# Sirui-Xu/InterDiff

Hardware: AMD Instinct MI355X
Metric: denoising frame-steps/sec (denoising-steps/sec x B x T frames) (higher is better)
Workload: dtype f32 (every contraction of the denoiser -- feed-forward block, QKV projection, self-attention, row-block contractions and the two token GEMMs: every fp32 operand as two f16 planes, 3 f16 MFMAs per product, fp32 accumulate; SMPL and everything else fp32 MFMA / VALU)

## Files before the change

### include/interdiff_hip.h

```cpp
#ifndef INTERDIFF_HIP_H
#define INTERDIFF_HIP_H

#include <stddef.h>
#include <stdint.h>

#ifdef __cplusplus
extern "C" {
#endif

#define IDF_OK            0
#define IDF_E_INVAL      -22
#define IDF_E_NOMEM      -12
#define IDF_E_LAUNCH     -5

int         interdiff_abi_version(void);
const char *interdiff_build_info(void);

int interdiff_rotation_6d_to_matrix   (const float *d6, float *m,  int64_t n, void *stream);
int interdiff_matrix_to_rotation_6d   (const float *m,  float *d6, int64_t n, void *stream);
int interdiff_matrix_to_axis_angle    (const float *m,  float *aa, int64_t n, void *stream);
int interdiff_axis_angle_to_matrix    (const float *aa, float *m,  int64_t n, void *stream);
int interdiff_axis_angle_to_quaternion(const float *aa, float *q,  int64_t n, void *stream);
int interdiff_rotation_6d_to_axis_angle(const float *d6, float *aa, int64_t n, void *stream);

// ... 160 lines not shown
size_t interdiff_correction_workspace_bytes(const idf_correction_ctx *c, int32_t B, int32_t T);
int interdiff_correction(const idf_correction_ctx *c, float *x0, const float *gt,
                         const float *hand_pose, const float *beta, const float *obj_points,
                         int32_t B, int32_t T, float blend_t ,
                         uint8_t *condition, int32_t *contact, float *distance, float *loss,
                         void *ws, size_t ws_bytes, void *stream);
int interdiff_correction_dev(const idf_correction_ctx *c, float *x0, const float *gt, const float *hand_pose,
                             const float *beta, const float *obj_points, int32_t B, int32_t T, const float *table,
                             const int64_t *state, void *ws, size_t ws_bytes, void *stream);

#define IDF_CONTACT_STATS 12
size_t interdiff_contact_nn_workspace_bytes(const idf_correction_ctx *c, int32_t B, int32_t T);
int interdiff_contact_nn(const idf_correction_ctx *c, const float *verts, const float *obj_points, const float *objR,
                         const float *objT, int32_t B, int32_t T, float *o2h, int32_t *idx, uint64_t *stats,
                         void *ws, size_t ws_bytes, void *stream);

size_t interdiff_metrics_workspace_bytes(const idf_correction_ctx *c, int32_t B, int32_t T);
int interdiff_metrics(const idf_correction_ctx *c, const float *obj_pred, const float *jtr,
                      const float *body_trans, const float *obj_gt, const float *jtr_gt,
                      const float *body_trans_gt, const float *verts, const float *obj_points,
                      int32_t B, int32_t T, int32_t J, float *out6 ,
                      void *ws, size_t ws_bytes, void *stream);

typedef struct {
    int32_t T, past_len, J, n_pre;
    const float *arena;
    int64_t dct_pad;
    int64_t dct;
    int64_t idct;
    int64_t layer[12];
// ... 113 lines not shown
```

### interdiff_amd/_lib.py

```python
import ctypes as C
import os
import torch

_HERE = os.path.dirname(os.path.abspath(__file__))
LIB_PATH = os.environ.get('INTERDIFF_HIP_LIB') or os.path.join(_HERE, 'csrc', 'libinterdiff_hip.so')
ABI_VERSION = 17

vp, i32, i64, f32, u64, sz = C.c_void_p, C.c_int32, C.c_int64, C.c_float, C.c_uint64, C.c_size_t

MDM_LAYERS = 8
FFN_SLICES = 5
STEP_EMBED_READY, STEP_EMBED_NEXT = 1, 2
LOSS_VAL, LOSS_TEST = 0, 1
TUNE = dict(ffn=3, ffn_math=4)


class SmplModel(C.Structure):
    _fields_ = [('V', i32), ('J', i32), ('n_betas', i32), ('KB', i32), ('S', i32),
                ('blend', vp), ('jt', vp), ('js', vp), ('parents', vp), ('skin_idx', vp), ('skin_w', vp)]


class MdmLayer(C.Structure):
    _fields_ = [('is_qan', i64),
                ('sa_in_w', i64), ('sa_in_b', i64), ('sa_out_w', i64), ('sa_out_b', i64),
# ... 91 lines not shown
    'interdiff_randn_at': (C.c_int, [vp, i64, u64, u64, u64, vp]),
    'interdiff_posterior_step_dev': (C.c_int, [vp, vp, vp, vp, i64, vp, vp, vp, i32, vp]),
    'interdiff_sampler_advance': (C.c_int, [vp, vp, i32, vp]),
    'interdiff_objprojector_sample': (C.c_int, [C.POINTER(ObjProj), vp, vp, vp, vp, i32, vp, vp]),
    'interdiff_objprojector_forward_workspace_bytes': (sz, [i32]),
    'interdiff_objprojector_forward': (C.c_int, [C.POINTER(ObjProj), vp, vp, vp, vp, i32, i32, vp, vp, sz, vp]),
    'interdiff_correction_workspace_bytes': (sz, [C.POINTER(CorrectionCtx), i32, i32]),
    'interdiff_correction': (C.c_int, [C.POINTER(CorrectionCtx), vp, vp, vp, vp, vp, i32, i32, f32,
                                       vp, vp, vp, vp, vp, sz, vp]),
    'interdiff_correction_dev': (C.c_int, [C.POINTER(CorrectionCtx), vp, vp, vp, vp, vp, i32, i32, vp, vp, vp, sz, vp]),
    'interdiff_metrics_workspace_bytes': (sz, [C.POINTER(CorrectionCtx), i32, i32]),
    'interdiff_metrics': (C.c_int, [C.POINTER(CorrectionCtx), vp, vp, vp, vp, vp, vp, vp, vp, i32, i32, i32,
                                    vp, vp, sz, vp]),
    'interdiff_contact_nn_workspace_bytes': (sz, [C.POINTER(CorrectionCtx), i32, i32]),
    'interdiff_contact_nn': (C.c_int, [C.POINTER(CorrectionCtx), vp, vp, vp, vp, i32, i32, vp, vp, vp, vp, sz, vp]),
    'interdiff_skeleton_objprojector_sample': (C.c_int, [C.POINTER(SkelObjProj), vp, vp, vp, i32, vp, vp, vp]),
    'interdiff_skeleton_correction': (C.c_int, [C.POINTER(SkelObjProj), vp, vp, vp, i32, i32, f32, vp, vp]),
    'interdiff_skeleton_metrics': (C.c_int, [vp, vp, vp, vp, vp, vp, i32, i32, i32, vp, vp]),
    'interdiff_skeleton_mdm_forward': (C.c_int, [C.POINTER(MdmWeights), C.POINTER(SkelHead), vp, vp, vp, vp, i32, i32, vp, vp, sz, vp]),
    'interdiff_skeleton_mdm_forward_step': (C.c_int, [C.POINTER(MdmWeights), C.POINTER(SkelHead), vp, vp, vp, vp, i32, i32, vp, vp, vp, vp, vp, sz, vp]),
    'interdiff_skeleton_mdm_encode_workspace_bytes': (sz, [i32, i32]),
    'interdiff_skeleton_mdm_encode': (C.c_int, [C.POINTER(MdmWeights), C.POINTER(SkelHead), vp, vp, i32, i32, vp, vp, sz, vp]),
    'interdiff_q_sample': (C.c_int, [vp, vp, vp, vp, vp, vp, i32, vp, vp, i32, i64, u64, u64, vp]),
    'interdiff_denoising_losses': (C.c_int, [vp, vp, i32, i32, i32, vp, vp]),
    'interdiff_sample_losses_workspace_bytes': (sz, [i32, i32]),
    'interdiff_sample_losses': (C.c_int, [vp, vp, vp, i32, i32, i32, i32, i32, vp, vp, vp, sz, vp]),
    'interdiff_correction_losses_workspace_bytes': (sz, [i32, i32, i32, i32]),
    'interdiff_correction_losses': (C.c_int, [vp, vp, vp, i32, vp, i32, i32, i32, i32, i32, i32, vp, vp, vp, sz, vp]),
    'interdiff_optimize_init': (C.c_int, [C.POINTER(OptCtx), C.POINTER(OptState), vp, vp, vp, vp, i32, vp]),
    'interdiff_optimize_loss_grad': (C.c_int, [C.POINTER(OptCtx), C.POINTER(OptState), vp]),
# ... 81 lines not shown
```

### interdiff_amd/correction.py

```python
import ctypes as C
import os
import itertools
import numpy as np
import torch
from . import _lib
from .geometry import MeshTopology

MARKERS67 = [3470, 3171, 3327, 857, 1812, 628, 182, 3116, 3040, 239,
             1666, 1725, 0, 2174, 1568, 1368, 3387, 2112, 1053, 1058,
             3336, 3346, 1323, 2108, 3122, 3314, 1252, 1082, 1861, 1454,
             850, 2224, 3233, 1769, 6728, 4343, 5273, 4116, 3694, 6399,
             6540, 6488, 3749, 5135, 5194, 3512, 5635, 5210, 4360, 4841,
             6786, 5573, 4538, 4544, 6736, 6747, 4804, 5568, 6544, 6682,
             5322, 4927, 5686, 4598, 6633, 3506, 3508]


_UID = itertools.count(1)


def correction_gate(t0):
    return not (t0 > 500 or t0 % 50 != 0)


class HipCorrection:
# ... 60 lines not shown
        hp, beta, pts = y['hand_pose'].contiguous().float(), y['beta'].contiguous().float(), y['obj_points'].contiguous().float()
        ws = self._workspace(B, T)
        dbg = [None] * 4
        if self.debug is not None:
            dbg = [torch.empty(B, dtype=torch.uint8, device=self.device), torch.empty(B, len(MARKERS67), dtype=torch.int32, device=self.device),
                   torch.empty(B, device=self.device), torch.empty(B, device=self.device)]
        blend_t = float(np.float32(t0) / np.float32(1000))
        _lib.check(self.lib.interdiff_correction(C.byref(self.ctx), _lib.dptr(x, torch.float32), _lib.dptr(gt, torch.float32),
                                                 _lib.dptr(hp), _lib.dptr(beta), _lib.dptr(pts), B, T, blend_t,
                                                 *[_lib.dptr(d, allow_none=True) for d in dbg], _lib.dptr(ws), ws.numel(),
                                                 _lib.stream()), 'correction')
        if self.debug is not None:
            self.debug.update(condition=dbg[0], contact=dbg[1], distance=dbg[2], loss=dbg[3])
        return x

    def contact_nn(self, verts, obj_points, objR, objT, want_stats=False):
        T, B = verts.shape[:2]
        P = self.ctx.n_points
        o2h = torch.empty(T, B, P, device=self.device)
        idx = torch.empty(T, B, P, dtype=torch.int32, device=self.device)
        stats = torch.zeros(12, dtype=torch.int64, device=self.device) if want_stats else None
        need = self.lib.interdiff_contact_nn_workspace_bytes(C.byref(self.ctx), B, T)
        ws = getattr(self, '_nn_ws', None)
        if ws is None or ws.numel() < need:
            ws = self._nn_ws = torch.empty(need, dtype=torch.uint8, device=self.device)
        v, pts, R_, t_ = (a.contiguous().float() for a in (verts, obj_points, objR, objT))
        _lib.check(self.lib.interdiff_contact_nn(C.byref(self.ctx), _lib.dptr(v), _lib.dptr(pts), _lib.dptr(R_), _lib.dptr(t_), B, T, _lib.dptr(o2h),
                                                 _lib.dptr(idx), _lib.dptr(stats, allow_none=True), _lib.dptr(ws), ws.numel(), _lib.stream()), 'contact_nn')
        return (o2h, idx, tuple(int(x) for x in stats.cpu())) if want_stats else (o2h, idx)

    def is_active(self, t0):
        return correction_gate(int(t0))

    def __call__(self, x, t, model_kwargs):
        t0 = getattr(t, 'host_value', None)
        if t0 is None:
            t0 = int(t[0])
        if not correction_gate(t0):
            return x
        return self.apply(x, t0, model_kwargs['y'])
```

### interdiff_amd/csrc/correction.hip

```cpp
#include "common.h"
#include "objproj.h"
#include "rot_math.h"
#include <float.h>

namespace {

constexpr int NBODY = 22;
constexpr int CTOK = 144;

__global__ __launch_bounds__(256) void corr_prepare_kernel(const float *__restrict__ x0, const float *__restrict__ gt,
                                                           const float *__restrict__ hand_pose, int B, int T,
                                                           float *__restrict__ pose, float *__restrict__ trans,
                                                           float *__restrict__ objR, float *__restrict__ objT,
                                                           float *__restrict__ gt_angles, float *__restrict__ gt_trans) {
    const int64_t i = (int64_t)blockIdx.x * 256 + threadIdx.x;
    const int64_t N = (int64_t)B * T;
    if (i >= N * 24) return;
    const int64_t n = i / 24;
    const int slot = (int)(i - n * 24), t = (int)(n / B), b = (int)(n - (int64_t)t * B);
    const float *xb = x0 + (size_t)b * CTOK * T + t;
    if (slot < NBODY) {
        float d[6], m[9], a[3];
#pragma unroll
        for (int k = 0; k < 6; ++k) d[k] = xb[(size_t)(slot * 6 + k) * T];
// ... 99 lines not shown
    }
#pragma unroll
    for (int k = 0; k < 2; ++k) {
        const int i = tid + 1024 * k;
        if (i < P) porder[(size_t)b * P + i] = (int32_t)(keys[i] & 2047u);
    }
}

constexpr int MAXM = 128;
constexpr float MARK_D2 = 0.00039999996079131961f;
constexpr int CB = 16;
constexpr int SB = 8;
constexpr int SEED_STRIDE = 4;
constexpr int CT = 1024;
constexpr int TASK = 64;
typedef float v2f __attribute__((ext_vector_type(2)));

struct ContactLds {
    int V4, nCB, nSB, nSeed;
    int rec, mark, box, sbox, seed, flags, red, pl, total;
    __host__ __device__ explicit ContactLds(int V) {
        V4 = (V + CB - 1) / CB * CB; nCB = V4 / CB; nSB = (nCB + SB - 1) / SB; nSeed = (nCB + SEED_STRIDE - 1) / SEED_STRIDE;
        rec = 0;
        mark = rec + V4;
        box = mark + MAXM;
        sbox = box + 3 * (nSB * SB / 2);
        seed = sbox + 3 * ((nSB + 2) / 2);
        flags = seed + 2 * ((nSeed + 1) / 2);
        red = flags + MAXM / 4;
        pl = red + CT / 4;
// ... 38 lines not shown
                                                          const int32_t *__restrict__ faces ,
                                                          const int32_t *__restrict__ adj_ptr,
                                                          const int32_t *__restrict__ adj_face,
                                                          const int32_t *__restrict__ adj_corner,
                                                          const int32_t *__restrict__ adj_pair ,
                                                          const int32_t *__restrict__ vorder ,
                                                          const int32_t *__restrict__ vrank ,
                                                          const int32_t *__restrict__ markers_pos , int M, int B,
                                                          float *__restrict__ markers_out, float *__restrict__ loss_sum,
                                                          float *__restrict__ min_dist, int32_t *__restrict__ label,
                                                          float *__restrict__ o2h_out ,
                                                          int32_t *__restrict__ idx_out ,
                                                          unsigned long long *__restrict__ stats ,
                                                          int64_t nn_from ,
                                                          const float *__restrict__ pts_frame , int frames_per_clip ,
                                                          const PredArgs pred) {
    extern __shared__ __attribute__((aligned(16))) float4 vs[];
    if constexpr (WITH_PRED) {
        if ((int)blockIdx.x < pred.nclips) {
            const int b = blockIdx.x, Tn = pred.op.T;
            for (int i = threadIdx.x; i < Tn * M; i += CT) {
                const int t = i / M, m = i - t * M;
                const size_t nfr = (size_t)t * B + b;
                const float *v = verts + (nfr * V + pred.markers_idx[m]) * 3;
                float *o = pred.markers + (nfr * M + m) * 3;
                o[0] = v[0]; o[1] = v[1]; o[2] = v[2];
            }
            __threadfence();
            __syncthreads();
            idf_objproj_dev::objproj_body<1>(reinterpret_cast<float *>(vs), pred.op, pred.obj_angles, pred.obj_trans, pred.markers, nullptr, B, b, pred.keep, nullptr);
            return;
        }
    }
    const ContactLds L(V);
    const int nCB = L.nCB, nSB = L.nSB;
    float4 *ms = vs + L.mark, *bb = vs + L.box, *sbb = vs + L.sbox, *sd = vs + L.seed;
    int *flags = reinterpret_cast<int *>(vs + L.flags);
    float *red = reinterpret_cast<float *>(vs + L.red);
    float *pl = reinterpret_cast<float *>(vs + L.pl);
    __shared__ int next_task;
    const int64_t n = WITH_PRED ? (int64_t)blockIdx.x - pred.nclips : (int64_t)blockIdx.x;
    const int b = OPT ? (int)(n / frames_per_clip) : (int)(n % B), tid = threadIdx.x;
    const float *vf = verts + (size_t)n * V * 3;
    const bool do_nn = n >= nn_from;
    long long t_prev = 0;
    int n_phase = 0;
    auto phase_done = [&]() {
        if (stats && tid == 0 && do_nn) {
            const long long now = (long long)__builtin_readcyclecounter();
            if (n_phase > 0) atomicAdd(stats + 3 + n_phase, (unsigned long long)(now - t_prev));
            t_prev = now;
        }
        ++n_phase;
    };
    phase_done();
    float R[9] = {1.f, 0.f, 0.f, 0.f, 1.f, 0.f, 0.f, 0.f, 1.f}, tr[3] = {0.f, 0.f, 0.f};
// ... 43 lines not shown
                typedef float f3v __attribute__((ext_vector_type(3), aligned(4)));
                const f3v pv = *reinterpret_cast<const f3v *>(vf + 3 * o[k]);
                x[k] = pv.x; y[k] = pv.y; z[k] = pv.z;
            }
        }
#pragma unroll
        for (int k = 0; k < 4; ++k) {
            const int v = v0 + k * CT;
            if (v < L.V4) {
                lds_rec_store(vs, v, x[k], y[k], z[k]);
                reinterpret_cast<int *>(vs + 2 * (v >> 1) + 1)[2 + (v & 1)] = o[k] >= 0 ? o[k] : 0x7fffffff;
            }
        }
    }
    if (tid < MAXM) flags[tid] = 0;
    const int ntask_all = (P + TASK - 1) / TASK;
    const int task0 = (int)((long long)blockIdx.y * ntask_all / gridDim.y), task1 = (int)((long long)(blockIdx.y + 1) * ntask_all / gridDim.y);
    if (tid == 0) next_task = task0;
    for (int i = tid; i < MAXP; i += CT) pl[i] = 0.f;
    __syncthreads();
    phase_done();
    if (!OPT && tid < ((M + 1) & ~1)) {
        float3 mk = make_float3(3e18f, 3e18f, 3e18f);
        if (tid < M) {
            mk = lds_rec(vs, my_marker_pos);
            if (markers_out) {
                float *mo = markers_out + ((size_t)n * M + tid) * 3;
                mo[0] = mk.x; mo[1] = mk.y; mo[2] = mk.z;
            }
        }
        lds_rec_store(ms, tid, mk.x, mk.y, mk.z);
// ... 21 lines not shown
            if ((lane_ & 7) == 0 && cb < nSB * SB) lds_box_store(bb, cb, make_float3(lx, ly, lz), make_float3(hx, hy, hz));
            const float slx = -wave_max(-lx), sly = -wave_max(-ly), slz = -wave_max(-lz), shx = wave_max(hx), shy = wave_max(hy), shz = wave_max(hz);
            if (lane_ == 0) lds_box_store(sbb, sb, make_float3(slx, sly, slz), make_float3(shx, shy, shz));
        }
#undef IDF_DPP8
        for (int k = tid; k < 2 * ((L.nSeed + 1) / 2); k += CT) {
            const float3 p = lds_rec(vs, min(k * SEED_STRIDE, nCB - 1) * CB);
            lds_rec_store(sd, k, p.x, p.y, p.z);
        }
    }
    const float *op = OPT ? pts_frame + (size_t)n * P * 3 : obj_points + (size_t)b * P * 3;
    const int ln = tid & 63, ntask = task1;
    __syncthreads();
    phase_done();
    float mind2 = FLT_MAX;
    unsigned n_exec = 0, n_test = 0, n_tasks = 0;
    for (;;) {
        int task = 0;
        if (ln == 0) task = atomicAdd(&next_task, 1);
        task = __builtin_amdgcn_readfirstlane(task);
        if (task >= ntask) break;
        ++n_tasks;
        const int sp = task * TASK + ln;
        const int i = sp < P ? (porder ? porder[(size_t)b * P + sp] : sp) : -1;
        const bool valid = i >= 0;
        float px = 0.f, py = 0.f, pz = 0.f;
        if (valid) { px = op[3 * i]; py = op[3 * i + 1]; pz = op[3 * i + 2]; }
        const float qx = OPT ? px : (px * R[0] + py * R[1] + pz * R[2]) + tr[0];
        const float qy = OPT ? py : (px * R[3] + py * R[4] + pz * R[5]) + tr[1];
        const float qz = OPT ? pz : (px * R[6] + py * R[7] + pz * R[8]) + tr[2];
        if (do_nn) {
#pragma clang fp contract(off)
            const v2f QX = v2f{qx, qx}, QY = v2f{qy, qy}, QZ = v2f{qz, qz};
            auto pair_d2 = [&](const float4 xy, const float4 zz) {
#pragma clang fp contract(off)
                const v2f dx = QX - v2f{xy.x, xy.y}, dy = QY - v2f{xy.z, xy.w}, dz = QZ - v2f{zz.x, zz.y};
                return (dx * dx + dy * dy) + dz * dz;
            };
            auto pair_a2 = [&](const float4 xy, const float2 zz) {
                const v2f dx = QX - v2f{xy.x, xy.y}, dy = QY - v2f{xy.z, xy.w}, dz = QZ - v2f{zz.x, zz.y};
                return __builtin_elementwise_fma(dz, dz, __builtin_elementwise_fma(dy, dy, dx * dx));
            };
            constexpr float SCAN_M = 1.000003814697265625f, SCAN_ABS = 1e-37f;
            float seed = FLT_MAX;
            for (int k = 0; k < (L.nSeed + 1) / 2; k += 4) {
                float4 xy[4]; float2 zz[4];
#pragma unroll
                for (int u = 0; u < 4; ++u) { xy[u] = sd[2 * min(k + u, (L.nSeed + 1) / 2 - 1)]; zz[u] = *reinterpret_cast<const float2 *>(&sd[2 * min(k + u, (L.nSeed + 1) / 2 - 1) + 1]); }
#pragma unroll
                for (int u = 0; u < 4; ++u) {
                    const v2f a2 = pair_a2(xy[u], zz[u]);
                    seed = fminf(fminf(seed, a2.x), a2.y);
                }
            }
            float thr = __builtin_fmaf(seed, SCAN_M, SCAN_ABS);
            float best = FLT_MAX, bthr = FLT_MAX;
            int tie = 0;
            int bblk = 0, bblk2 = 0;
            auto pair_lb = [&](const float4 a, const float4 bq, const float4 c) {
#pragma clang fp contract(off)
                const v2f ax = v2f{a.x, a.y} - QX, bx = QX - v2f{bq.z, bq.w};
                const v2f ay = v2f{a.z, a.w} - QY, by = QY - v2f{c.x, c.y};
                const v2f az = v2f{bq.x, bq.y} - QZ, bz = QZ - v2f{c.z, c.w};
                const v2f ex = v2f{fmaxf(fmaxf(ax.x, bx.x), 0.f), fmaxf(fmaxf(ax.y, bx.y), 0.f)};
                const v2f ey = v2f{fmaxf(fmaxf(ay.x, by.x), 0.f), fmaxf(fmaxf(ay.y, by.y), 0.f)};
                const v2f ez = v2f{fmaxf(fmaxf(az.x, bz.x), 0.f), fmaxf(fmaxf(az.y, bz.y), 0.f)};
                return __builtin_elementwise_fma(ez, ez, __builtin_elementwise_fma(ey, ey, ex * ex));
            };
            auto score_block = [&](int cb) {
                ++n_exec;
                const int v0 = cb * CB;
                float4 xy[CB / 2]; float2 zz[CB / 2];
#pragma unroll
                for (int u = 0; u < CB / 2; ++u) { xy[u] = vs[v0 + 2 * u]; zz[u] = *reinterpret_cast<const float2 *>(&vs[v0 + 2 * u + 1]); }
                float bm = FLT_MAX;
#pragma unroll
                for (int u = 0; u < CB / 2; ++u) {
                    const v2f a2 = pair_a2(xy[u], zz[u]);
                    bm = fminf(fminf(bm, a2.x), a2.y);
                }
                if (bm < best) {
                    const float w = __builtin_fmaf(bm, SCAN_M, SCAN_ABS);
                    if (best <= w) { tie = tie ? 2 : 1; bblk2 = bblk; } else tie = 0;
                    best = bm; bblk = v0; bthr = w; thr = fminf(thr, w);
                } else if (bm <= bthr) { tie = tie ? 2 : 1; bblk2 = v0; }
            };
            auto scan_super = [&](int sb) {
                const int cb0 = sb * SB;
#pragma unroll
                for (int j = 0; j < SB / 2; ++j) {
                    const int cb = cb0 + 2 * j;
                    const float4 *bx = bb + 3 * (cb >> 1);
                    const v2f lb = pair_lb(bx[0], bx[1], bx[2]);
                    n_test += 2;
                    if (__builtin_amdgcn_ballot_w64(valid && lb.x <= thr) != 0ull) score_block(cb);
                    if (__builtin_amdgcn_ballot_w64(valid && lb.y <= thr) != 0ull) score_block(cb + 1);
                }
            };
            if (!vorder) {
                for (int cb = 0; cb < nCB; ++cb) score_block(cb);
            } else
            for (int sb = 0; sb < nSB; sb += 2) {
                const float4 *bx = sbb + 3 * (sb >> 1);
                const v2f lb = pair_lb(bx[0], bx[1], bx[2]);
                n_test += 2;
                if (__builtin_amdgcn_ballot_w64(valid && lb.x <= thr) != 0ull) scan_super(sb);
                if (__builtin_amdgcn_ballot_w64(valid && lb.y <= thr) != 0ull) scan_super(sb + 1);
            }
            int pos = bblk, org = 0x7fffffff;
            float ebest = FLT_MAX;
            auto resolve_pair = [&](int pr) {
                const float4 xy = vs[2 * pr], zz = vs[2 * pr + 1];
                const v2f d2 = pair_d2(xy, zz);
                const int o0 = __builtin_bit_cast(int, zz.z), o1 = __builtin_bit_cast(int, zz.w);
                if (d2.x < ebest || (d2.x == ebest && o0 < org)) { ebest = d2.x; org = o0; pos = 2 * pr; }
                if (d2.y < ebest || (d2.y == ebest && o1 < org)) { ebest = d2.y; org = o1; pos = 2 * pr + 1; }
            };
            if (tie < 2) {
#pragma unroll
                for (int u = 0; u < CB / 2; ++u) resolve_pair((bblk >> 1) + u);
                if (tie) {
#pragma unroll
                    for (int u = 0; u < CB / 2; ++u) resolve_pair((bblk2 >> 1) + u);
                }
            } else {
                for (int pr = 0; pr < (V + 1) / 2; ++pr) resolve_pair(pr);
            }
            pos = min(pos, V - 1);
            if (org == 0x7fffffff) org = vorder ? vorder[pos] : pos;
            if constexpr (OPT) {
                if (valid) idx_out[(size_t)n * P + i] = org;
            } else if (valid) {
                const float3 v3 = lds_rec(vs, pos);
                float3 acc = make_float3(0.f, 0.f, 0.f);
                const int e0 = adj_ptr[org], e1 = adj_ptr[org + 1];
                if (adj_pair) {
                    for (int e = e0; e < e1; e += 4) {
                        int2 ab[4];
#pragma unroll
                        for (int u = 0; u < 4; ++u) ab[u] = *reinterpret_cast<const int2 *>(adj_pair + 2 * (size_t)min(e + u, e1 - 1));
#pragma unroll
                        for (int u = 0; u < 4; ++u) {
                            if (e + u < e1) {
                                const float3 nn = cross3(sub3(lds_rec(vs, ab[u].x), v3), sub3(lds_rec(vs, ab[u].y), v3));
                                acc.x += nn.x; acc.y += nn.y; acc.z += nn.z;
                            }
// ... 3 lines not shown
                    for (int e = e0; e < e1; ++e) {
                        const int f = adj_face[e], c = adj_corner[e];
                        const float3 p0 = lds_rec(vs, faces[3 * f]), p1 = lds_rec(vs, faces[3 * f + 1]), p2 = lds_rec(vs, faces[3 * f + 2]);
                        float3 nn;
                        if (c == 1) nn = cross3(sub3(p2, p1), sub3(p0, p1));
                        else if (c == 2) nn = cross3(sub3(p0, p2), sub3(p1, p2));
                        else nn = cross3(sub3(p1, p0), sub3(p2, p0));
                        acc.x += nn.x; acc.y += nn.y; acc.z += nn.z;
                    }
                }
                const float nl = fmaxf(sqrtf(acc.x * acc.x + acc.y * acc.y + acc.z * acc.z), 1e-6f);
                const float vx = qx - v3.x, vy = qy - v3.y, vz = qz - v3.z;
                const float dt = (acc.x / nl) * vx + (acc.y / nl) * vy + (acc.z / nl) * vz;
                const float d = sqrtf(vx * vx + vy * vy + vz * vz);
                const float o2h = d * (dt > 0.f ? 1.f : (dt < 0.f ? -1.f : 0.f));
                if (o2h_out) o2h_out[(size_t)n * P + i] = o2h;
                if (idx_out) idx_out[(size_t)n * P + i] = org;
                pl[sp] = o2h < 0.f ? fabsf(o2h) * 20.0f : 0.f;
            }
        }
        if (!OPT && valid) {
#pragma clang fp contract(off)
            const v2f QX = v2f{qx, qx}, QY = v2f{qy, qy}, QZ = v2f{qz, qz};
            for (int p2 = 0; p2 < (M + 1) / 2; ++p2) {
                const float4 xy = ms[2 * p2], zz = ms[2 * p2 + 1];
                const v2f dx = v2f{xy.x, xy.y} - QX, dy = v2f{xy.z, xy.w} - QY, dz = v2f{zz.x, zz.y} - QZ;
                const v2f d2 = __builtin_elementwise_fma(dy, dy, dx * dx) + dz * dz;
                mind2 = fminf(fminf(mind2, d2.x), d2.y);
                if (__builtin_amdgcn_ballot_w64(fminf(d2.x, d2.y) < MARK_D2) != 0ull) {
                    if (d2.x < MARK_D2) flags[2 * p2] = 1;
                    if (d2.y < MARK_D2) flags[2 * p2 + 1] = 1;
                }
            }
        }
    }
    if (stats && ln == 0 && do_nn) {
        atomicAdd(stats, (unsigned long long)n_exec);
        atomicAdd(stats + 1, (unsigned long long)nCB * n_tasks);
        atomicAdd(stats + 2, (unsigned long long)n_test);
    }
    phase_done();
    if constexpr (OPT) return;
    __syncthreads();
    phase_done();
    float loss = 0.f;
#pragma unroll
    for (int k = 0; k < MAXP / CT; ++k) loss += pl[tid + CT * k];
    red[tid] = loss;
    __syncthreads();
    for (int s = CT / 2; s > 0; s >>= 1) {
        if (tid < s) red[tid] += red[tid + s];
        __syncthreads();
    }
    const float loss_total = red[0];
// ... 5 lines not shown
        __syncthreads();
    }
    if (tid == 0) { loss_sum[n] = loss_total; min_dist[n] = red[0] == FLT_MAX ? FLT_MAX : sqrtf(red[0]); }
    if (tid < M) label[(size_t)n * M + tid] = flags[tid];
    phase_done();
    if (stats && tid == 0 && do_nn) atomicAdd(stats + 3, 1ull);
}

size_t contact_lds_bytes(int V) { return (size_t)ContactLds(V).total * sizeof(float4); }

int launch_contact(hipStream_t s, int64_t N, const float *verts, int V, const float *obj_points, int P, int32_t *porder,
                   const float *objR, const float *objT, const idf_correction_ctx *c, int B, float *markers, float *loss_sum,
                   float *min_dist, int32_t *label, float *o2h, int32_t *idx, unsigned long long *stats, int64_t nn_from, const PredArgs *pred = nullptr) {
    const int M = c->n_markers;
    const size_t lds = contact_lds_bytes(V);
    if (lds > 160 * 1024 - 16384 || P > MAXP) return IDF_E_INVAL;
    const bool ordered = c->vorder != nullptr;
    if (ordered != (c->faces_scan != nullptr) || ordered != (c->markers_scan != nullptr) || ordered != (c->adj_pair_scan != nullptr)) return IDF_E_INVAL;
    const int32_t *faces = ordered ? c->faces_scan : c->faces, *mpos = ordered ? c->markers_scan : c->markers_idx;
    if (porder) hipLaunchKernelGGL(corr_point_order_kernel, dim3((unsigned)B), dim3(1024), 0, s, obj_points, P, porder);
    if (pred) {
        const size_t lds2 = (pred->nclips > 0 && lds < idf_objproj_dev::OBJPROJ_LDS) ? idf_objproj_dev::OBJPROJ_LDS : lds;
        static std::atomic<uint64_t> lds_ok2{0};
        if (lds2 > 160 * 1024 - 2048) return IDF_E_INVAL;
        if (idf_opt_in_lds(reinterpret_cast<const void *>(corr_contact_kernel<false, true>), 160 * 1024 - 2048, lds_ok2) != IDF_OK) return IDF_E_LAUNCH;
        hipLaunchKernelGGL((corr_contact_kernel<false, true>), dim3((unsigned)(N + pred->nclips)), dim3(CT), lds2, s, verts, V, obj_points, P, porder, objR, objT, faces,
                           c->adj_ptr, c->adj_face, c->adj_corner, c->adj_pair_scan, c->vorder, c->vrank, mpos, M, B, markers, loss_sum, min_dist, label, o2h, idx,
                           stats, nn_from, nullptr, 0, *pred);
        return IDF_OK;
    }
    static std::atomic<uint64_t> lds_ok{0};
    if (idf_opt_in_lds(reinterpret_cast<const void *>(corr_contact_kernel<false>), 160 * 1024 - 16384, lds_ok) != IDF_OK) return IDF_E_LAUNCH;
    hipLaunchKernelGGL(corr_contact_kernel<false>, dim3((unsigned)N), dim3(CT), lds, s, verts, V, obj_points, P, porder, objR, objT, faces,
                       c->adj_ptr, c->adj_face, c->adj_corner, c->adj_pair_scan, c->vorder, c->vrank, mpos, M, B, markers, loss_sum, min_dist, label, o2h, idx,
                       stats, nn_from, nullptr, 0, PredArgs{});
    return IDF_OK;
}

__global__ __launch_bounds__(128) void corr_reduce_kernel(const float *__restrict__ loss_sum, const float *__restrict__ min_dist,
                                                          const int32_t *__restrict__ label, int B, int T, int past, int P, int M,
                                                          uint8_t *__restrict__ condition, int32_t *__restrict__ contact,
                                                          float *__restrict__ distance_out, float *__restrict__ loss_out) {
    extern __shared__ float fr[];
    const int b = blockIdx.x, tid = threadIdx.x;
    for (int t = tid; t < T; t += 128) {
        fr[t] = loss_sum[(size_t)t * B + b];
        fr[T + t] = min_dist[(size_t)t * B + b];
    }
    if (tid < M) {
        int c = 0;
// ... 129 lines not shown
    }
    if (valid) near[(size_t)n * V + vid] = hit ? 1 : 0;
}

}

int idf_point_order(hipStream_t s, const float *obj_points, int B, int P, int32_t *porder) {
    if (P > MAXP) return IDF_E_INVAL;
    hipLaunchKernelGGL(corr_point_order_kernel, dim3((unsigned)B), dim3(1024), 0, s, obj_points, P, porder);
    return IDF_OK;
}

int idf_nn_scan_opt(hipStream_t s, int64_t N, int frames_per_clip, const float *verts, int V, const float *pts_frame, const float *obj_points, int P,
                    const int32_t *porder, const idf_correction_ctx *c, int32_t *yidx) {
    const size_t lds = contact_lds_bytes(V);
    if (lds > 160 * 1024 - 16384 || P > MAXP || !c->vorder) return IDF_E_INVAL;
    const int B = (int)(N / frames_per_clip);
    static std::atomic<uint64_t> lds_ok{0};
    if (idf_opt_in_lds(reinterpret_cast<const void *>(corr_contact_kernel<true>), 160 * 1024 - 16384, lds_ok) != IDF_OK) return IDF_E_LAUNCH;
    hipLaunchKernelGGL(corr_contact_kernel<true>, dim3((unsigned)N, 2), dim3(CT), lds, s, verts, V, obj_points, P, porder, nullptr, nullptr, nullptr,
                       nullptr, nullptr, nullptr, nullptr, c->vorder, c->vrank, nullptr, 0, B, nullptr, nullptr, nullptr, nullptr, nullptr, yidx, nullptr, (int64_t)0,
                       pts_frame, frames_per_clip, PredArgs{});
    return IDF_OK;
}

int idf_near_mask_opt(hipStream_t s, int64_t N, int frames_per_clip, const float *verts, int V, const float *pts_frame, int P, const int32_t *porder,
                      const int32_t *vorder, float *psort, float *pbox, int32_t *near) {
    if (P > MAXP || !vorder) return IDF_E_INVAL;
    hipLaunchKernelGGL(opt_patch_kernel, dim3((unsigned)N), dim3(256), 0, s, pts_frame, P, porder, frames_per_clip, reinterpret_cast<float4 *>(psort),
                       reinterpret_cast<float4 *>(pbox));
    hipLaunchKernelGGL(opt_near_kernel, dim3((unsigned)idf_cdiv(V, 256), (unsigned)N), dim3(256), 0, s, verts, V, P, reinterpret_cast<const float4 *>(psort),
                       reinterpret_cast<const float4 *>(pbox), vorder, near);
    return IDF_OK;
}

namespace {

}

extern "C" size_t interdiff_correction_workspace_bytes(const idf_correction_ctx *c, int32_t B, int32_t T) {
    if (!c || !c->smpl || B <= 0 || T <= 0) return 0;
    return carve(c, B, T, nullptr).total;
}

static int correction_impl(const idf_correction_ctx *c, float *x0, const float *gt, const float *hand_pose,
                           const float *beta, const float *obj_points, int32_t B, int32_t T, float blend_t, const float *blend_table,
                           const int64_t *blend_state, uint8_t *condition, int32_t *contact, float *distance, float *loss, void *ws,
                           size_t ws_bytes, void *stream) {
    if (!c || !c->smpl || !c->objproj || !x0 || !gt || !hand_pose || !beta || !obj_points || !ws || B <= 0 || T <= 0) return IDF_E_INVAL;
    const int V = c->smpl->V, M = c->n_markers, P = c->n_points;
    if (c->smpl->J != 52 || c->smpl->n_betas != 10 || M > MAXM || M != c->objproj->P || P > MAXP || T != c->objproj->T ||
        c->past_len != c->objproj->past_len || c->past_len >= T)
        return IDF_E_INVAL;
    CorrWs w = carve(c, B, T, ws);
    if (ws_bytes < w.total) return IDF_E_NOMEM;
    hipStream_t s = idf_stream(stream);
    const int64_t N = (int64_t)B * T;
    const bool fused = (c->tune & 2) == 0 && idf_objproj_check(c->objproj) == IDF_OK;
    idf_prof_mark(IDF_K_CORR_PREPARE, s);
    hipLaunchKernelGGL(corr_prepare_kernel, dim3((unsigned)idf_cdiv(N * 24, 256)), dim3(256), 0, s, x0, gt, hand_pose, B, T, w.pose,
                       w.trans, w.objR, w.objT, w.gt_angles, w.gt_trans);
    int rc = interdiff_smpl_forward(c->smpl, w.pose, beta, w.trans, N, w.verts, w.jtr, nullptr, w.smpl_ws, w.smpl_ws_bytes, stream);
    if (rc) return rc;
    idf_prof_mark(IDF_K_CORR_CONTACT, s);
    PredArgs pred{};
    if (fused) {
        pred.op = *c->objproj;
// ... 145 lines not shown
    if (!c || B <= 0 || T <= 0) return 0;
    return carve_metrics(c, B, T, nullptr).total;
}

extern "C" int interdiff_contact_nn(const idf_correction_ctx *c, const float *verts, const float *obj_points, const float *objR,
                                    const float *objT, int32_t B, int32_t T, float *o2h, int32_t *idx, uint64_t *stats, void *ws,
                                    size_t ws_bytes, void *stream) {
    if (!c || !c->smpl || !verts || !obj_points || !objR || !objT || !ws || B <= 0 || T <= 0 || (!o2h && !idx)) return IDF_E_INVAL;
    if (c->n_markers > MAXM || c->n_points > MAXP) return IDF_E_INVAL;
    MetWs w = carve_metrics(c, B, T, ws);
    if (ws_bytes < w.total) return IDF_E_NOMEM;
    hipStream_t s = idf_stream(stream);
    if (stats && hipMemsetAsync(stats, 0, IDF_CONTACT_STATS * sizeof(uint64_t), s) != hipSuccess) return IDF_E_LAUNCH;
    const int rc = launch_contact(s, (int64_t)B * T, verts, c->smpl->V, obj_points, c->n_points, w.porder, objR, objT, c, B, w.markers, w.loss_sum,
                                  w.min_dist, w.label, o2h ? o2h : w.o2h, idx, reinterpret_cast<unsigned long long *>(stats), 0);
    if (rc) return rc;
    IDF_CHECK_LAUNCH();
    return IDF_OK;
}

extern "C" size_t interdiff_metrics_workspace_bytes(const idf_correction_ctx *c, int32_t B, int32_t T) {
    if (!c || B <= 0 || T <= 0) return 0;
    return carve_metrics(c, B, T, nullptr).total;
}

extern "C" int interdiff_metrics(const idf_correction_ctx *c, const float *obj_pred, const float *jtr, const float *body_trans,
                                 const float *obj_gt, const float *jtr_gt, const float *body_trans_gt, const float *verts,
                                 const float *obj_points, int32_t B, int32_t T, int32_t J, float *out6, void *ws, size_t ws_bytes,
                                 void *stream) {
    if (!c || !c->smpl || !obj_pred || !jtr || !body_trans || !obj_gt || !jtr_gt || !body_trans_gt || !verts || !obj_points || !out6 ||
// ... 20 lines not shown
```

Measured before the change: 7.317 million.

## Split each contact nearest-neighbour query across two lanes with DPP reductions

Adds a two-lane mode, on by default, to the contact kernel. Each object point is handled by a lane pair: the seed scan, block scoring and exhaustive rescans are split between the two lanes, and the partial minima and argmins are combined through DPP swaps. This halves the points per task and aims to shorten the serial per-point scan and cut divergence, at the cost of more ballots and cross-lane shuffles. The change also reorders workgroups so that nearest-neighbour frames launch first, raises the opt-in LDS limit, adds runner and rescan statistics, and exposes a standalone contact_nn_opt entry point.

```diff
diff --git a/include/interdiff_hip.h b/include/interdiff_hip.h
--- a/include/interdiff_hip.h
+++ b/include/interdiff_hip.h
@@ -198,6 +198,9 @@
 int interdiff_contact_nn(const idf_correction_ctx *c, const float *verts, const float *obj_points, const float *objR,
                          const float *objT, int32_t B, int32_t T, float *o2h, int32_t *idx, uint64_t *stats,
                          void *ws, size_t ws_bytes, void *stream);
+
+int interdiff_contact_nn_opt(const idf_correction_ctx *c, const float *verts, const float *pts_frame, const float *obj_points, int32_t B,
+                             int32_t T, int32_t *porder, int32_t *idx, void *stream);
 
 size_t interdiff_metrics_workspace_bytes(const idf_correction_ctx *c, int32_t B, int32_t T);
 int interdiff_metrics(const idf_correction_ctx *c, const float *obj_pred, const float *jtr,
diff --git a/interdiff_amd/_lib.py b/interdiff_amd/_lib.py
--- a/interdiff_amd/_lib.py
+++ b/interdiff_amd/_lib.py
@@ -129,6 +129,7 @@
                                     vp, vp, sz, vp]),
     'interdiff_contact_nn_workspace_bytes': (sz, [C.POINTER(CorrectionCtx), i32, i32]),
     'interdiff_contact_nn': (C.c_int, [C.POINTER(CorrectionCtx), vp, vp, vp, vp, i32, i32, vp, vp, vp, vp, sz, vp]),
+    'interdiff_contact_nn_opt': (C.c_int, [C.POINTER(CorrectionCtx), vp, vp, vp, i32, i32, vp, vp, vp]),
     'interdiff_skeleton_objprojector_sample': (C.c_int, [C.POINTER(SkelObjProj), vp, vp, vp, i32, vp, vp, vp]),
     'interdiff_skeleton_correction': (C.c_int, [C.POINTER(SkelObjProj), vp, vp, vp, i32, i32, f32, vp, vp]),
     'interdiff_skeleton_metrics': (C.c_int, [vp, vp, vp, vp, vp, vp, i32, i32, i32, vp, vp]),
diff --git a/interdiff_amd/correction.py b/interdiff_amd/correction.py
--- a/interdiff_amd/correction.py
+++ b/interdiff_amd/correction.py
@@ -98,7 +98,7 @@
             self.debug.update(condition=dbg[0], contact=dbg[1], distance=dbg[2], loss=dbg[3])
         return x
 
-    def contact_nn(self, verts, obj_points, objR, objT, want_stats=False):
+    def contact_nn(self, verts, obj_points, objR, objT, want_stats=False, want_frames=False):
         T, B = verts.shape[:2]
         P = self.ctx.n_points
         o2h = torch.empty(T, B, P, device=self.device)
@@ -111,7 +111,29 @@
         v, pts, R_, t_ = (a.contiguous().float() for a in (verts, obj_points, objR, objT))
         _lib.check(self.lib.interdiff_contact_nn(C.byref(self.ctx), _lib.dptr(v), _lib.dptr(pts), _lib.dptr(R_), _lib.dptr(t_), B, T, _lib.dptr(o2h),
                                                  _lib.dptr(idx), _lib.dptr(stats, allow_none=True), _lib.dptr(ws), ws.numel(), _lib.stream()), 'contact_nn')
-        return (o2h, idx, tuple(int(x) for x in stats.cpu())) if want_stats else (o2h, idx)
+        out = (o2h, idx)
+        if want_stats:
+            out += (tuple(int(x) for x in stats.cpu()),)
+        if want_frames:
+            N, M, al = T * B, self.ctx.n_markers, lambda x: (x + 255) // 256 * 256
+            off = al(N * 36) + al(N * 12) + al(N * P * 4) + al(N * M * 12)
+            loss_sum = ws[off:off + N * 4].view(torch.float32).reshape(T, B).clone()
+            off += al(N * 4)
+            min_dist = ws[off:off + N * 4].view(torch.float32).reshape(T, B).clone()
+            off += al(N * 4)
+            label = ws[off:off + N * M * 4].view(torch.int32).reshape(T, B, M).clone()
+            out += (dict(loss_sum=loss_sum, min_dist=min_dist, label=label),)
+        return out
+
+    def contact_nn_opt(self, verts, pts_frame, obj_points):
+        B, T = verts.shape[:2]
+        P = self.ctx.n_points
+        idx = torch.empty(B, T, P, dtype=torch.int32, device=self.device)
+        porder = torch.empty(B, P, dtype=torch.int32, device=self.device)
+        v, pf, pts = (a.contiguous().float() for a in (verts, pts_frame, obj_points))
+        _lib.check(self.lib.interdiff_contact_nn_opt(C.byref(self.ctx), _lib.dptr(v), _lib.dptr(pf), _lib.dptr(pts), B, T, _lib.dptr(porder), _lib.dptr(idx),
+                                                     _lib.stream()), 'contact_nn_opt')
+        return idx
 
     def is_active(self, t0):
         return correction_gate(int(t0))
diff --git a/interdiff_amd/csrc/correction.hip b/interdiff_amd/csrc/correction.hip
--- a/interdiff_amd/csrc/correction.hip
+++ b/interdiff_amd/csrc/correction.hip
@@ -137,6 +137,7 @@
 constexpr int SEED_STRIDE = 4;
 constexpr int CT = 1024;
 constexpr int TASK = 64;
+constexpr size_t CONTACT_LDS_MAX = 160 * 1024 - 2048;
 typedef float v2f __attribute__((ext_vector_type(2)));
 
 struct ContactLds {
@@ -205,6 +206,7 @@
                                                           unsigned long long *__restrict__ stats ,
                                                           int64_t nn_from ,
                                                           const float *__restrict__ pts_frame , int frames_per_clip ,
+                                                          int two_lane ,
                                                           const PredArgs pred) {
     extern __shared__ __attribute__((aligned(16))) float4 vs[];
     if constexpr (WITH_PRED) {
@@ -230,7 +232,9 @@
     float *red = reinterpret_cast<float *>(vs + L.red);
     float *pl = reinterpret_cast<float *>(vs + L.pl);
     __shared__ int next_task;
-    const int64_t n = WITH_PRED ? (int64_t)blockIdx.x - pred.nclips : (int64_t)blockIdx.x;
+    const int64_t wg = WITH_PRED ? (int64_t)blockIdx.x - pred.nclips : (int64_t)blockIdx.x;
+    const int64_t n_frames = (int64_t)gridDim.x - (WITH_PRED ? pred.nclips : 0), n_scan = n_frames - nn_from;
+    const int64_t n = (nn_from > 0 && n_scan > 0) ? (wg < n_scan ? wg + nn_from : wg - n_scan) : wg;
     const int b = OPT ? (int)(n / frames_per_clip) : (int)(n % B), tid = threadIdx.x;
     const float *vf = verts + (size_t)n * V * 3;
     const bool do_nn = n >= nn_from;
@@ -304,7 +308,8 @@
         }
     }
     if (tid < MAXM) flags[tid] = 0;
-    const int ntask_all = (P + TASK - 1) / TASK;
+    const int task_pts = two_lane ? TASK / 2 : TASK;
+    const int ntask_all = (P + task_pts - 1) / task_pts;
     const int task0 = (int)((long long)blockIdx.y * ntask_all / gridDim.y), task1 = (int)((long long)(blockIdx.y + 1) * ntask_all / gridDim.y);
     if (tid == 0) next_task = task0;
     for (int i = tid; i < MAXP; i += CT) pl[i] = 0.f;
@@ -356,14 +361,18 @@
     __syncthreads();
     phase_done();
     float mind2 = FLT_MAX;
-    unsigned n_exec = 0, n_test = 0, n_tasks = 0;
+    unsigned n_exec = 0, n_test = 0, n_tasks = 0, n_runner = 0, n_rescan = 0;
+    const int hl = two_lane ? (ln & 1) : 0;
+    const unsigned long long lanes_first = two_lane ? 0x5555555555555555ull : ~0ull;
+    auto other_f = [](float v) { return __builtin_bit_cast(float, __builtin_amdgcn_update_dpp(0, __builtin_bit_cast(int, v), 0xB1, 0xf, 0xf, false)); };
+    auto other_i = [](int v) { return __builtin_amdgcn_update_dpp(0, v, 0xB1, 0xf, 0xf, false); };
     for (;;) {
         int task = 0;
         if (ln == 0) task = atomicAdd(&next_task, 1);
         task = __builtin_amdgcn_readfirstlane(task);
         if (task >= ntask) break;
         ++n_tasks;
-        const int sp = task * TASK + ln;
+        const int sp = two_lane ? task * (TASK / 2) + (ln >> 1) : task * TASK + ln;
         const int i = sp < P ? (porder ? porder[(size_t)b * P + sp] : sp) : -1;
         const bool valid = i >= 0;
         float px = 0.f, py = 0.f, pz = 0.f;
@@ -385,7 +394,7 @@
             };
             constexpr float SCAN_M = 1.000003814697265625f, SCAN_ABS = 1e-37f;
             float seed = FLT_MAX;
-            for (int k = 0; k < (L.nSeed + 1) / 2; k += 4) {
+            auto seed_group = [&](int k) {
                 float4 xy[4]; float2 zz[4];
 #pragma unroll
                 for (int u = 0; u < 4; ++u) { xy[u] = sd[2 * min(k + u, (L.nSeed + 1) / 2 - 1)]; zz[u] = *reinterpret_cast<const float2 *>(&sd[2 * min(k + u, (L.nSeed + 1) / 2 - 1) + 1]); }
@@ -394,6 +403,12 @@
                     const v2f a2 = pair_a2(xy[u], zz[u]);
                     seed = fminf(fminf(seed, a2.x), a2.y);
                 }
+            };
+            if (two_lane) {
+                for (int k = 4 * hl; k < (L.nSeed + 1) / 2; k += 8) seed_group(k);
+                seed = fminf(seed, other_f(seed));
+            } else {
+                for (int k = 0; k < (L.nSeed + 1) / 2; k += 4) seed_group(k);
             }
             float thr = __builtin_fmaf(seed, SCAN_M, SCAN_ABS);
             float best = FLT_MAX, bthr = FLT_MAX;
@@ -409,23 +424,40 @@
                 const v2f ez = v2f{fmaxf(fmaxf(az.x, bz.x), 0.f), fmaxf(fmaxf(az.y, bz.y), 0.f)};
                 return __builtin_elementwise_fma(ez, ez, __builtin_elementwise_fma(ey, ey, ex * ex));
             };
-            auto score_block = [&](int cb) {
-                ++n_exec;
-                const int v0 = cb * CB;
-                float4 xy[CB / 2]; float2 zz[CB / 2];
-#pragma unroll
-                for (int u = 0; u < CB / 2; ++u) { xy[u] = vs[v0 + 2 * u]; zz[u] = *reinterpret_cast<const float2 *>(&vs[v0 + 2 * u + 1]); }
-                float bm = FLT_MAX;
-#pragma unroll
-                for (int u = 0; u < CB / 2; ++u) {
-                    const v2f a2 = pair_a2(xy[u], zz[u]);
-                    bm = fminf(fminf(bm, a2.x), a2.y);
-                }
+            auto block_scored = [&](float bm, int v0) {
                 if (bm < best) {
                     const float w = __builtin_fmaf(bm, SCAN_M, SCAN_ABS);
                     if (best <= w) { tie = tie ? 2 : 1; bblk2 = bblk; } else tie = 0;
                     best = bm; bblk = v0; bthr = w; thr = fminf(thr, w);
                 } else if (bm <= bthr) { tie = tie ? 2 : 1; bblk2 = v0; }
+            };
+            auto score_block = [&](int cb) {
+                ++n_exec;
+                const int v0 = cb * CB;
+                float4 xy[CB / 2]; float2 zz[CB / 2];
+#pragma unroll
+                for (int u = 0; u < CB / 2; ++u) { xy[u] = vs[v0 + 2 * u]; zz[u] = *reinterpret_cast<const float2 *>(&vs[v0 + 2 * u + 1]); }
+                float bm = FLT_MAX;
+#pragma unroll
+                for (int u = 0; u < CB / 2; ++u) {
+                    const v2f a2 = pair_a2(xy[u], zz[u]);
+                    bm = fminf(fminf(bm, a2.x), a2.y);
+                }
+                block_scored(bm, v0);
+            };
+            auto score_block2 = [&](int cb) {
+                ++n_exec;
+                const int v0 = cb * CB, h0 = v0 + (CB / 2) * hl;
+                float4 xy[CB / 4]; float2 zz[CB / 4];
+#pragma unroll
+                for (int u = 0; u < CB / 4; ++u) { xy[u] = vs[h0 + 2 * u]; zz[u] = *reinterpret_cast<const float2 *>(&vs[h0 + 2 * u + 1]); }
+                float bm = FLT_MAX;
+#pragma unroll
+                for (int u = 0; u < CB / 4; ++u) {
+                    const v2f a2 = pair_a2(xy[u], zz[u]);
+                    bm = fminf(fminf(bm, a2.x), a2.y);
+                }
+                block_scored(fminf(bm, other_f(bm)), v0);
             };
             auto scan_super = [&](int sb) {
                 const int cb0 = sb * SB;
@@ -439,8 +471,35 @@
                     if (__builtin_amdgcn_ballot_w64(valid && lb.y <= thr) != 0ull) score_block(cb + 1);
                 }
             };
+            constexpr unsigned long long EVEN = 0x5555555555555555ull, ODD = 0xaaaaaaaaaaaaaaaaull;
+            auto scan_super2 = [&](int sb) {
+                const int cb0 = sb * SB;
+#pragma unroll
+                for (int j = 0; j < SB / 4; ++j) {
+                    const int cb = cb0 + 4 * j;
+                    const float4 *bx = bb + 3 * ((cb >> 1) + hl);
+                    const v2f lb = pair_lb(bx[0], bx[1], bx[2]);
+                    n_test += 4;
+                    if ((__builtin_amdgcn_ballot_w64(valid && lb.x <= thr) & EVEN) != 0ull) score_block2(cb);
+                    if ((__builtin_amdgcn_ballot_w64(valid && lb.y <= thr) & EVEN) != 0ull) score_block2(cb + 1);
+                    if ((__builtin_amdgcn_ballot_w64(valid && lb.x <= thr) & ODD) != 0ull) score_block2(cb + 2);
+                    if ((__builtin_amdgcn_ballot_w64(valid && lb.y <= thr) & ODD) != 0ull) score_block2(cb + 3);
+                }
+            };
             if (!vorder) {
-                for (int cb = 0; cb < nCB; ++cb) score_block(cb);
+                if (two_lane) for (int cb = 0; cb < nCB; ++cb) score_block2(cb);
+                else for (int cb = 0; cb < nCB; ++cb) score_block(cb);
+            } else if (two_lane) {
+                const int nsbp = (nSB + 2) / 2;
+                for (int sb = 0; sb < nSB; sb += 4) {
+                    const float4 *bx = sbb + 3 * min((sb >> 1) + hl, nsbp - 1);
+                    const v2f lb = pair_lb(bx[0], bx[1], bx[2]);
+                    n_test += 4;
+                    if ((__builtin_amdgcn_ballot_w64(valid && lb.x <= thr) & EVEN) != 0ull) scan_super2(sb);
+                    if (sb + 1 < nSB && (__builtin_amdgcn_ballot_w64(valid && lb.y <= thr) & EVEN) != 0ull) scan_super2(sb + 1);
+                    if (sb + 2 < nSB && (__builtin_amdgcn_ballot_w64(valid && lb.x <= thr) & ODD) != 0ull) scan_super2(sb + 2);
+                    if (sb + 3 < nSB && (__builtin_amdgcn_ballot_w64(valid && lb.y <= thr) & ODD) != 0ull) scan_super2(sb + 3);
+                }
             } else
             for (int sb = 0; sb < nSB; sb += 2) {
                 const float4 *bx = sbb + 3 * (sb >> 1);
@@ -458,7 +517,23 @@
                 if (d2.x < ebest || (d2.x == ebest && o0 < org)) { ebest = d2.x; org = o0; pos = 2 * pr; }
                 if (d2.y < ebest || (d2.y == ebest && o1 < org)) { ebest = d2.y; org = o1; pos = 2 * pr + 1; }
             };
-            if (tie < 2) {
+            n_runner += (unsigned)__builtin_popcountll(__builtin_amdgcn_ballot_w64(valid && tie == 1) & lanes_first);
+            n_rescan += (unsigned)__builtin_popcountll(__builtin_amdgcn_ballot_w64(valid && tie == 2) & lanes_first);
+            if (two_lane) {
+                if (tie < 2) {
+#pragma unroll
+                    for (int u = 0; u < CB / 4; ++u) resolve_pair((bblk >> 1) + (CB / 4) * hl + u);
+                    if (tie) {
+#pragma unroll
+                        for (int u = 0; u < CB / 4; ++u) resolve_pair((bblk2 >> 1) + (CB / 4) * hl + u);
+                    }
+                } else {
+                    for (int pr = hl; pr < (V + 1) / 2; pr += 2) resolve_pair(pr);
+                }
+                const float oe = other_f(ebest);
+                const int oo = other_i(org), opos = other_i(pos);
+                if (oe < ebest || (oe == ebest && (oo < org || (oo == org && opos < pos)))) { ebest = oe; org = oo; pos = opos; }
+            } else if (tie < 2) {
 #pragma unroll
                 for (int u = 0; u < CB / 2; ++u) resolve_pair((bblk >> 1) + u);
                 if (tie) {
@@ -471,7 +546,7 @@
             pos = min(pos, V - 1);
             if (org == 0x7fffffff) org = vorder ? vorder[pos] : pos;
             if constexpr (OPT) {
-                if (valid) idx_out[(size_t)n * P + i] = org;
+                if (valid && hl == 0) idx_out[(size_t)n * P + i] = org;
             } else if (valid) {
                 const float3 v3 = lds_rec(vs, pos);
                 float3 acc = make_float3(0.f, 0.f, 0.f);
@@ -505,15 +580,15 @@
                 const float dt = (acc.x / nl) * vx + (acc.y / nl) * vy + (acc.z / nl) * vz;
                 const float d = sqrtf(vx * vx + vy * vy + vz * vz);
                 const float o2h = d * (dt > 0.f ? 1.f : (dt < 0.f ? -1.f : 0.f));
-                if (o2h_out) o2h_out[(size_t)n * P + i] = o2h;
-                if (idx_out) idx_out[(size_t)n * P + i] = org;
-                pl[sp] = o2h < 0.f ? fabsf(o2h) * 20.0f : 0.f;
+                if (o2h_out && hl == 0) o2h_out[(size_t)n * P + i] = o2h;
+                if (idx_out && hl == 0) idx_out[(size_t)n * P + i] = org;
+                if (hl == 0) pl[sp] = o2h < 0.f ? fabsf(o2h) * 20.0f : 0.f;
             }
         }
         if (!OPT && valid) {
 #pragma clang fp contract(off)
             const v2f QX = v2f{qx, qx}, QY = v2f{qy, qy}, QZ = v2f{qz, qz};
-            for (int p2 = 0; p2 < (M + 1) / 2; ++p2) {
+            for (int p2 = hl; p2 < (M + 1) / 2; p2 += two_lane ? 2 : 1) {
                 const float4 xy = ms[2 * p2], zz = ms[2 * p2 + 1];
                 const v2f dx = v2f{xy.x, xy.y} - QX, dy = v2f{xy.z, xy.w} - QY, dz = v2f{zz.x, zz.y} - QZ;
                 const v2f d2 = __builtin_elementwise_fma(dy, dy, dx * dx) + dz * dz;
@@ -529,6 +604,8 @@
         atomicAdd(stats, (unsigned long long)n_exec);
         atomicAdd(stats + 1, (unsigned long long)nCB * n_tasks);
         atomicAdd(stats + 2, (unsigned long long)n_test);
+        atomicAdd(stats + 9, (unsigned long long)n_runner);
+        atomicAdd(stats + 10, (unsigned long long)n_rescan);
     }
     phase_done();
     if constexpr (OPT) return;
@@ -564,7 +641,8 @@
                    float *min_dist, int32_t *label, float *o2h, int32_t *idx, unsigned long long *stats, int64_t nn_from, const PredArgs *pred = nullptr) {
     const int M = c->n_markers;
     const size_t lds = contact_lds_bytes(V);
-    if (lds > 160 * 1024 - 16384 || P > MAXP) return IDF_E_INVAL;
+    if (lds > CONTACT_LDS_MAX || P > MAXP) return IDF_E_INVAL;
+    const int two_lane = (c->tune & 4) == 0;
     const bool ordered = c->vorder != nullptr;
     if (ordered != (c->faces_scan != nullptr) || ordered != (c->markers_scan != nullptr) || ordered != (c->adj_pair_scan != nullptr)) return IDF_E_INVAL;
     const int32_t *faces = ordered ? c->faces_scan : c->faces, *mpos = ordered ? c->markers_scan : c->markers_idx;
@@ -572,18 +650,18 @@
     if (pred) {
         const size_t lds2 = (pred->nclips > 0 && lds < idf_objproj_dev::OBJPROJ_LDS) ? idf_objproj_dev::OBJPROJ_LDS : lds;
         static std::atomic<uint64_t> lds_ok2{0};
-        if (lds2 > 160 * 1024 - 2048) return IDF_E_INVAL;
-        if (idf_opt_in_lds(reinterpret_cast<const void *>(corr_contact_kernel<false, true>), 160 * 1024 - 2048, lds_ok2) != IDF_OK) return IDF_E_LAUNCH;
+        if (lds2 > CONTACT_LDS_MAX) return IDF_E_INVAL;
+        if (idf_opt_in_lds(reinterpret_cast<const void *>(corr_contact_kernel<false, true>), (int)CONTACT_LDS_MAX, lds_ok2) != IDF_OK) return IDF_E_LAUNCH;
         hipLaunchKernelGGL((corr_contact_kernel<false, true>), dim3((unsigned)(N + pred->nclips)), dim3(CT), lds2, s, verts, V, obj_points, P, porder, objR, objT, faces,
                            c->adj_ptr, c->adj_face, c->adj_corner, c->adj_pair_scan, c->vorder, c->vrank, mpos, M, B, markers, loss_sum, min_dist, label, o2h, idx,
-                           stats, nn_from, nullptr, 0, *pred);
+                           stats, nn_from, nullptr, 0, two_lane, *pred);
         return IDF_OK;
     }
     static std::atomic<uint64_t> lds_ok{0};
-    if (idf_opt_in_lds(reinterpret_cast<const void *>(corr_contact_kernel<false>), 160 * 1024 - 16384, lds_ok) != IDF_OK) return IDF_E_LAUNCH;
+    if (idf_opt_in_lds(reinterpret_cast<const void *>(corr_contact_kernel<false>), (int)CONTACT_LDS_MAX, lds_ok) != IDF_OK) return IDF_E_LAUNCH;
     hipLaunchKernelGGL(corr_contact_kernel<false>, dim3((unsigned)N), dim3(CT), lds, s, verts, V, obj_points, P, porder, objR, objT, faces,
                        c->adj_ptr, c->adj_face, c->adj_corner, c->adj_pair_scan, c->vorder, c->vrank, mpos, M, B, markers, loss_sum, min_dist, label, o2h, idx,
-                       stats, nn_from, nullptr, 0, PredArgs{});
+                       stats, nn_from, nullptr, 0, two_lane, PredArgs{});
     return IDF_OK;
 }
 
@@ -743,13 +821,13 @@
 int idf_nn_scan_opt(hipStream_t s, int64_t N, int frames_per_clip, const float *verts, int V, const float *pts_frame, const float *obj_points, int P,
                     const int32_t *porder, const idf_correction_ctx *c, int32_t *yidx) {
     const size_t lds = contact_lds_bytes(V);
-    if (lds > 160 * 1024 - 16384 || P > MAXP || !c->vorder) return IDF_E_INVAL;
+    if (lds > CONTACT_LDS_MAX || P > MAXP || !c->vorder) return IDF_E_INVAL;
     const int B = (int)(N / frames_per_clip);
     static std::atomic<uint64_t> lds_ok{0};
-    if (idf_opt_in_lds(reinterpret_cast<const void *>(corr_contact_kernel<true>), 160 * 1024 - 16384, lds_ok) != IDF_OK) return IDF_E_LAUNCH;
+    if (idf_opt_in_lds(reinterpret_cast<const void *>(corr_contact_kernel<true>), (int)CONTACT_LDS_MAX, lds_ok) != IDF_OK) return IDF_E_LAUNCH;
     hipLaunchKernelGGL(corr_contact_kernel<true>, dim3((unsigned)N, 2), dim3(CT), lds, s, verts, V, obj_points, P, porder, nullptr, nullptr, nullptr,
                        nullptr, nullptr, nullptr, nullptr, c->vorder, c->vrank, nullptr, 0, B, nullptr, nullptr, nullptr, nullptr, nullptr, yidx, nullptr, (int64_t)0,
-                       pts_frame, frames_per_clip, PredArgs{});
+                       pts_frame, frames_per_clip, (c->tune & 4) == 0 ? 1 : 0, PredArgs{});
     return IDF_OK;
 }
 
@@ -779,7 +857,7 @@
     if (!c || !c->smpl || !c->objproj || !x0 || !gt || !hand_pose || !beta || !obj_points || !ws || B <= 0 || T <= 0) return IDF_E_INVAL;
     const int V = c->smpl->V, M = c->n_markers, P = c->n_points;
     if (c->smpl->J != 52 || c->smpl->n_betas != 10 || M > MAXM || M != c->objproj->P || P > MAXP || T != c->objproj->T ||
-        c->past_len != c->objproj->past_len || c->past_len >= T)
+        c->past_len != c->objproj->past_len || c->past_len >= T || contact_lds_bytes(V) > CONTACT_LDS_MAX)
         return IDF_E_INVAL;
     CorrWs w = carve(c, B, T, ws);
     if (ws_bytes < w.total) return IDF_E_NOMEM;
@@ -955,6 +1033,17 @@
     if (stats && hipMemsetAsync(stats, 0, IDF_CONTACT_STATS * sizeof(uint64_t), s) != hipSuccess) return IDF_E_LAUNCH;
     const int rc = launch_contact(s, (int64_t)B * T, verts, c->smpl->V, obj_points, c->n_points, w.porder, objR, objT, c, B, w.markers, w.loss_sum,
                                   w.min_dist, w.label, o2h ? o2h : w.o2h, idx, reinterpret_cast<unsigned long long *>(stats), 0);
+    if (rc) return rc;
+    IDF_CHECK_LAUNCH();
+    return IDF_OK;
+}
+
+extern "C" int interdiff_contact_nn_opt(const idf_correction_ctx *c, const float *verts, const float *pts_frame, const float *obj_points, int32_t B,
+                                        int32_t T, int32_t *porder, int32_t *idx, void *stream) {
+    if (!c || !c->smpl || !verts || !pts_frame || !obj_points || !porder || !idx || B <= 0 || T <= 0) return IDF_E_INVAL;
+    hipStream_t s = idf_stream(stream);
+    if (contact_lds_bytes(c->smpl->V) > CONTACT_LDS_MAX || idf_point_order(s, obj_points, B, c->n_points, porder) != IDF_OK) return IDF_E_INVAL;
+    const int rc = idf_nn_scan_opt(s, (int64_t)B * T, T, verts, c->smpl->V, pts_frame, obj_points, c->n_points, porder, c, idx);
     if (rc) return rc;
     IDF_CHECK_LAUNCH();
     return IDF_OK;
```

Measured after the change: 7.218 million. 0.986x the previous value.
